# kiwicampus/multicamera_stitching

Hardware: NVIDIA B200
Metric: panoramas_per_sec (higher is better)
Workload: dtype u8

## Files before the change

multicamera_stitching_b200/csrc/mcs_stitch_tiled.cu:

```cuda
#include "mcs_device.cuh"

#include <cuda.h>
#include <string.h>
#include <stdlib.h>

#define TILED_WARPS MCS_TILED_WARPS
#define TILED_THREADS (32 * TILED_WARPS)
#define TILED_MIN_CTAS 2
#define TILED_PX_BATCH 4
#define TILED_SMEM_BUDGET_KB 113
#define TILED_MAX_STAGES 8
#define TILED_LOOKAHEAD_SLACK 2

struct TiledArgs {
    CUtensorMap tmap[MCS_MAX_LAYERS];
    const McsTile* tiles;
    const int4* issue;
    const McsLayer* layers;
    const uint32_t* desc;
    uint8_t* dst;
    long long dst_pitch;
    long long dst_frame_stride;
    int box_bytes;
    int stages;
    unsigned* work;
    int claim;
    int n_tiles;
    int n_chunks;
    int chunks_per_block;
    int split_first, split_end, split;
    int light_every, light_end, heavy_end, n_heavy;
    int frame_block;
    int nf_last;
    int n_blocks;
    int class_first[MCS_N_CLASSES + 1];
    int layer_sp[MCS_MAX_LAYERS];
    int layer_ox[MCS_MAX_LAYERS];
    const uint8_t* fast;
    int fast_stride;
    int fast_passes;
    int use_fast;
    const int4* band_issue;
    const uint32_t* band_desc;
    int feather_log2;
    int ov_bytes;
};

extern __shared__ __align__(128) uint8_t smem[];

__device__ __forceinline__ uint32_t smem_u32(const void* p) {
    return (uint32_t)__cvta_generic_to_shared(p);
}
__device__ __forceinline__ void mbar_init(uint32_t bar, int count) {
    asm volatile("mbarrier.init.shared::cta.b64 [%0], %1;" ::"r"(bar), "r"(count));
}
__device__ __forceinline__ void mbar_expect_tx(uint32_t bar, uint32_t bytes) {
    asm volatile("mbarrier.arrive.expect_tx.shared::cta.b64 _, [%0], %1;" ::"r"(bar), "r"(bytes) : "memory");
}
__device__ __forceinline__ void mbar_arrive(uint32_t bar) {
    asm volatile("mbarrier.arrive.shared::cta.b64 _, [%0];" ::"r"(bar) : "memory");
}
#ifdef TILED_DEBUG_HANG
#define TILED_HANG_CHECK(n_, what_)                                                                              \
    if (++(n_) > (1u << 26)) {                                                                                   \
        printf("tiled kernel stuck: %s line %d cta %d thread %d\n", what_, __LINE__, blockIdx.x, threadIdx.x);  \
        __trap();                                                                                                \
    }
#else
#define TILED_HANG_CHECK(n_, what_)
#endif
__device__ __forceinline__ void mbar_wait(uint32_t bar, uint32_t parity, int line = 0) {
    uint32_t done;
#ifdef TILED_DEBUG_HANG
    unsigned spins = 0;
#endif
    do {
        asm volatile(
            "{\n\t.reg .pred p;\n\t"
            "mbarrier.try_wait.parity.shared::cta.b64 p, [%1], %2;\n\t"
            "selp.u32 %0, 1, 0, p;\n\t}"
            : "=r"(done)
            : "r"(bar), "r"(parity)
            : "memory");
#ifdef TILED_DEBUG_HANG
        if (!done && ++spins > (1u << 22)) {
            printf("tiled kernel stuck: mbarrier wait from line %d cta %d thread %d bar %u parity %u\n", line, blockIdx.x,
                   threadIdx.x, bar, parity);
            __trap();
        }
#endif
    } while (!done);
}
__device__ __forceinline__ void tma_load_3d(uint32_t smem_dst, const CUtensorMap* map, int c0, int c1, int c2,
                                            uint32_t bar) {
    asm volatile(
        "cp.async.bulk.tensor.3d.shared::cluster.global.tile.mbarrier::complete_tx::bytes "
        "[%0], [%1, {%2, %3, %4}], [%5];" ::"r"(smem_dst),
        "l"(reinterpret_cast<uint64_t>(map)), "r"(c0), "r"(c1), "r"(c2), "r"(bar)
        : "memory");
}
__device__ __forceinline__ void bulk_g2s(uint32_t smem_dst, const void* src, uint32_t bytes, uint32_t bar) {
    asm volatile("cp.async.bulk.shared::cluster.global.mbarrier::complete_tx::bytes [%0], [%1], %2, [%3];" ::"r"(smem_dst),
                 "l"(src), "r"(bytes), "r"(bar)
                 : "memory");
}
__device__ __forceinline__ void cp_async16(uint32_t smem_dst, const void* src) {
    asm volatile("cp.async.ca.shared.global [%0], [%1], 16;" ::"r"(smem_dst), "l"(src) : "memory");
}
__device__ __forceinline__ void cp_async_wait_all() { asm volatile("cp.async.wait_all;" ::: "memory"); }
__device__ __forceinline__ uint32_t lds32(uint32_t addr) {
    uint32_t v;
    asm volatile("ld.shared.b32 %0, [%1];" : "=r"(v) : "r"(addr));
    return v;
}
__device__ __forceinline__ uint32_t lds32_box(uint32_t addr) {
    uint32_t v;
    asm("ld.shared.b32 %0, [%1];" : "=r"(v) : "r"(addr));
    return v;
}
__device__ __forceinline__ uint32_t order_after_wait(uint32_t addr) {
    asm volatile("" : "+r"(addr)::"memory");
    return addr;
}
__device__ __forceinline__ uint4 lds128(uint32_t addr) {
    uint4 v;
    asm volatile("ld.shared.v4.b32 {%0, %1, %2, %3}, [%4];" : "=r"(v.x), "=r"(v.y), "=r"(v.z), "=r"(v.w) : "r"(addr));
    return v;
}
__device__ __forceinline__ uint2 lds64(uint32_t addr) {
    uint2 v;
    asm volatile("ld.shared.v2.b32 {%0, %1}, [%2];" : "=r"(v.x), "=r"(v.y) : "r"(addr));
    return v;
}
__device__ __forceinline__ uint32_t lds8(uint32_t addr) {
    uint32_t v;
    asm volatile("ld.shared.u8 %0, [%1];" : "=r"(v) : "r"(addr));
    return v;
}
__device__ __forceinline__ uint32_t lds16(uint32_t addr) {
    uint32_t v;
    asm volatile("ld.shared.u16 %0, [%1];" : "=r"(v) : "r"(addr));
    return v;
}
__device__ __forceinline__ void sts8(uint32_t addr, uint32_t v) {
    asm volatile("st.shared.u8 [%0], %1;" ::"r"(addr), "r"(v) : "memory");
}
__device__ __forceinline__ void sts16(uint32_t addr, uint32_t v) {
    asm volatile("st.shared.u16 [%0], %1;" ::"r"(addr), "h"((unsigned short)v) : "memory");
}
__device__ __forceinline__ void sts32(uint32_t addr, uint32_t v) {
    asm volatile("st.shared.b32 [%0], %1;" ::"r"(addr), "r"(v) : "memory");
}
__device__ __forceinline__ uint32_t dp2a_lo(uint32_t w, uint32_t p, uint32_t acc) {
    uint32_t r;
    asm("dp2a.lo.u32.u32 %0, %1, %2, %3;" : "=r"(r) : "r"(w), "r"(p), "r"(acc));
    return r;
}
__device__ __forceinline__ uint32_t dp2a_hi(uint32_t w, uint32_t p, uint32_t acc) {
    uint32_t r;
    asm("dp2a.hi.u32.u32 %0, %1, %2, %3;" : "=r"(r) : "r"(w), "r"(p), "r"(acc));
    return r;
}
__device__ __forceinline__ uint32_t prmt(uint32_t a, uint32_t b, uint32_t sel) {
    uint32_t r;
    asm("prmt.b32 %0, %1, %2, %3;" : "=r"(r) : "r"(a), "r"(b), "r"(sel));
    return r;
}

#define MCS_STG128(p, v) __stcs((p), (v))

#define TILED_QD 32
#define TILED_SCHED_LEAD 10
struct SchedMem {
    int published;
    int pre_k;
    int pad[2];
    int4 pre;
    int4 pre_ov[MCS_BAND_MAX_OVERLAYS];
    int4 cur_ov[MCS_BAND_MAX_OVERLAYS];
// ... 239 lines not shown
        const uint32_t lo0 = __funnelshift_r(u0, u1, d.sh), lo1 = __funnelshift_r(v0, v1, d.sh);
        t[0] = dp2a_lo(d.w1, lo1, dp2a_lo(d.w0, lo0, 32768u));
    }
}

__device__ __forceinline__ PxDesc expand_desc(uint32_t w) {
    PxDesc d;
    const uint32_t b = w & 0xffffu, ax = (w >> 16) & 31u, ay = (w >> 21) & 31u;
    const uint32_t iax64 = (32u - ax) << 6, ax64 = ax << 6, iay = 32u - ay;
    d.off = b & ~3u;
    d.sh = b << 3;
    d.w0 = min(65535u, iay * iax64) | ((iay * ax64) << 16);
    d.w1 = (ay * iax64) | ((ay * ax64) << 16);
    return d;
}

struct RowOut {
    uint32_t s_chunk;
    uint32_t sh;
    uint32_t s_byte;
    uint32_t g_chunk;
    uint32_t g_byte;
    bool do_chunk, do_byte;
};

__device__ __forceinline__ RowOut row_split(uint32_t s_first, uint32_t g_first, uint32_t g_phase, bool has,
                                            int nbytes, int lane) {
    RowOut r;
    const int al = (int)((16u - g_phase) & 15u);
    const int head = min(nbytes, al);
    const int n = has ? (nbytes - head) >> 4 : 0;
    r.do_chunk = lane < n;
    r.s_chunk = s_first + al + (lane << 4);
    r.sh = 0;
    r.g_chunk = g_first + al + (lane << 4);
    const int e = lane < 16 ? lane : head + (n << 4) + lane - 16;
    r.do_byte = has && (lane < 16 ? lane < head : e < nbytes);
    r.s_byte = s_first + e;
    r.g_byte = g_first + e;
    return r;
}

__device__ __forceinline__ void write_out(const RowOut& r0, const RowOut& r1, bool ragged, uint8_t* frame) {
    const uint4 v0 = lds128(r0.s_chunk);
    const uint4 v1 = lds128(r1.s_chunk);
    if (r0.do_chunk) MCS_STG128(reinterpret_cast<uint4*>(frame + r0.g_chunk), v0);
    if (r1.do_chunk) MCS_STG128(reinterpret_cast<uint4*>(frame + r1.g_chunk), v1);
    if (ragged) {
        if (r0.do_byte) frame[r0.g_byte] = (uint8_t)lds8(r0.s_byte);
        if (r1.do_byte) frame[r1.g_byte] = (uint8_t)lds8(r1.s_byte);
    }
}

__device__ __forceinline__ void copy_out(const RowOut& r, uint32_t box, bool ragged, uint8_t* frame) {
    if (r.do_chunk) {
        const uint32_t w = box + r.s_chunk;
        const uint32_t w0 = lds32(w), w1 = lds32(w + 4), w2 = lds32(w + 8), w3 = lds32(w + 12), w4 = lds32(w + 16);
        uint4 v;
        v.x = __funnelshift_r(w0, w1, r.sh);
        v.y = __funnelshift_r(w1, w2, r.sh);
        v.z = __funnelshift_r(w2, w3, r.sh);
        v.w = __funnelshift_r(w3, w4, r.sh);
        MCS_STG128(reinterpret_cast<uint4*>(frame + r.g_chunk), v);
    }
    if (ragged && r.do_byte) frame[r.g_byte] = (uint8_t)lds8(box + r.s_byte);
}

template <int C>
__device__ __forceinline__ void stage_px(uint32_t o16, uint32_t o8, const uint32_t (&t)[C]) {
    if (C == 3) {
        sts16(o16, __byte_perm(t[0], t[1], 0x0062));
        sts8(o8, t[2] >> 16);
    } else {
#pragma unroll
        for (int k = 0; k < C; ++k) sts8(o16 + k, t[k] >> 16);
    }
}

#define TILED_SCHED_BYTES 640
static_assert(sizeof(SchedMem) <= TILED_SCHED_BYTES, "SchedMem must fit its shared-memory slot");

#define TILED_DESC_BUF_BYTES (MCS_FAST_HEADER_BYTES + MCS_CELL_W * MCS_CELL_H * 4)
static_assert(MCS_FAST_GROUP_BYTES + MCS_FAST_MAX_PASSES * MCS_FAST_PASS_BYTES <= MCS_CELL_W * MCS_CELL_H * 4,
              "a FAST record must fit the chunk-record buffer");

struct RingPos {
    int slot;
    uint32_t phase;
    int n;
    __device__ __forceinline__ void advance(int stages) {
        ++n;
        if (++slot == stages) { slot = 0; phase ^= 1; }
    }
};

struct Smem {
    uint32_t base;
    uint32_t out;
    uint32_t full;
    uint32_t empty;
    uint32_t dbar;
    uint32_t dbuf;
    uint32_t ov;
    SchedMem* issuer;
};

__device__ __forceinline__ void prefetch_chunk(const TiledArgs& a, const Smem& sm, int b, int4 e) {
    const int t = e.x;
    sts32(sm.dbar + 32 + 16 * b, (uint32_t)e.y);
    sts32(sm.dbar + 36 + 16 * b, (uint32_t)e.z);
    sts32(sm.dbar + 40 + 16 * b, (uint32_t)e.w);
    const int cls = tile_class(a, t);
    const uint32_t dst = sm.dbuf + b * TILED_DESC_BUF_BYTES, bar = sm.dbar + 8 * b;
    if (cls == MCS_TILE_FAST && a.use_fast) {
        mbar_expect_tx(bar, (uint32_t)a.fast_stride);
        bulk_g2s(dst, a.fast + (size_t)(t - a.class_first[1]) * a.fast_stride, (uint32_t)a.fast_stride, bar);
    } else if (cls >= MCS_TILE_WARP) {
        mbar_expect_tx(bar, 32u + MCS_CELL_W * MCS_CELL_H * 4u);
        bulk_g2s(dst, a.tiles + t, 32u, bar);
        bulk_g2s(dst + MCS_FAST_HEADER_BYTES, a.desc + (size_t)t * (MCS_CELL_W * MCS_CELL_H), MCS_CELL_W * MCS_CELL_H * 4u, bar);
    } else {
        mbar_expect_tx(bar, 32u);
        bulk_g2s(dst, a.tiles + t, 32u, bar);
    }
}

template <int C, int SP, bool ISS, bool BAND, bool BANDS>
__device__ __forceinline__ void warp_frames(const TiledArgs& a, const PxDesc (&d)[8], uint32_t groups, uint32_t sp,
                                            const Smem& sm, RingPos& ring, Issuer& issuer, int k_cons, uint8_t* frame,
                                            uint32_t g_row0, int n_fr, int c0, int nbytes, int h, int warp,
                                            int lane, int n_ov = 0, uint32_t ov_sp0 = 0, uint32_t ov_sp1 = 0,
                                            bool zero_base = false) {
    uint32_t ov_slots = 0;
    if (BAND) {
        for (int o = 0; o < n_ov; ++o)
#pragma unroll
            for (int j = 0; j < 8; ++j) {
                const uint32_t w = lds32(sm.ov + (uint32_t)o * (MCS_CELL_W * MCS_CELL_H * 4) + ((j * TILED_WARPS + warp) * 32 + lane) * 4);
                if (__any_sync(0xffffffffu, (w >> 26) != 0u)) ov_slots |= 1u << (8 * o + j);
            }
    }
    constexpr int OUT_PITCH = MCS_CELL_W * C + 16;
    const int stages = a.stages;
    const uint32_t g_row1 = g_row0 + (uint32_t)TILED_WARPS * (uint32_t)a.dst_pitch;
    const uint32_t s_row0 = sm.out + warp * OUT_PITCH, s_row1 = s_row0 + TILED_WARPS * OUT_PITCH;
    const bool has0 = warp < h, has1 = warp + TILED_WARPS < h;
    const bool phase_moves = (a.dst_frame_stride & 15) != 0;

    uint32_t ph0 = ((uint32_t)reinterpret_cast<uintptr_t>(frame) + g_row0) & 15u;
    uint32_t ph1 = ((uint32_t)reinterpret_cast<uintptr_t>(frame) + g_row1) & 15u;
    RowOut r0 = row_split(s_row0 + ph0 + c0 * C, g_row0 + c0 * C, (ph0 + c0 * C) & 15u, has0, nbytes, lane);
    RowOut r1 = row_split(s_row1 + ph1 + c0 * C, g_row1 + c0 * C, (ph1 + c0 * C) & 15u, has1, nbytes, lane);
    uint32_t st0 = s_row0 + ph0 + lane * C, st1 = s_row1 + ph1 + lane * C;
    uint32_t par = C == 3 ? (st0 & 1u) : 0u;
    TapSel sel = tap_sel<C>(par);
    bool ragged = __any_sync(0xffffffffu, r0.do_byte || r1.do_byte);

    for (int i = 0; i < n_fr; ++i, frame += a.dst_frame_stride) {
        if (ISS && lane == 0) issuer_step<BANDS, BAND>(a, sm.issuer, issuer, k_cons, ring.n, sm.base, sm.full, sm.empty);
        if (phase_moves && i != 0) {
            ph0 = ((uint32_t)reinterpret_cast<uintptr_t>(frame) + g_row0) & 15u;
            ph1 = ((uint32_t)reinterpret_cast<uintptr_t>(frame) + g_row1) & 15u;
            r0 = row_split(s_row0 + ph0 + c0 * C, g_row0 + c0 * C, (ph0 + c0 * C) & 15u, has0, nbytes, lane);
            r1 = row_split(s_row1 + ph1 + c0 * C, g_row1 + c0 * C, (ph1 + c0 * C) & 15u, has1, nbytes, lane);
            st0 = s_row0 + ph0 + lane * C;
            st1 = s_row1 + ph1 + lane * C;
            ragged = __any_sync(0xffffffffu, r0.do_byte || r1.do_byte);
            if (C == 3) {
                par = st0 & 1u;
                sel = tap_sel<C>(par);
            }
        }
        const uint32_t o16_0 = st0 + par, o8_0 = st0 + 2 - 2 * par;
        const uint32_t o16_1 = st1 + par, o8_1 = st1 + 2 - 2 * par;

        if (BAND && zero_base) {
            uint32_t z[C];
#pragma unroll
            for (int k = 0; k < C; ++k) z[k] = 0u;
#pragma unroll
            for (int j8 = 0; j8 < 8; ++j8) {
                const int g = 32 * (j8 & 3) * C;
                stage_px<C>((j8 < 4 ? o16_0 : o16_1) + g, (j8 < 4 ? o8_0 : o8_1) + g, z);
            }
            __syncwarp();
        } else {
        mbar_wait(sm.full + 8 * ring.slot, ring.phase, __LINE__);
        const uint32_t box = order_after_wait(sm.base + ring.slot * a.box_bytes);
        if (groups == 0xffu) {
#pragma unroll
            for (int b = 0; b < 8; b += TILED_PX_BATCH) {
                uint32_t t[TILED_PX_BATCH][C];
#pragma unroll
                for (int j = 0; j < TILED_PX_BATCH; ++j) sample_px<C, SP>(box, sp, d[b + j], sel, t[j]);
#pragma unroll
                for (int j = 0; j < TILED_PX_BATCH; ++j) {
                    const int g = 32 * ((b + j) & 3) * C;
                    stage_px<C>((b + j < 4 ? o16_0 : o16_1) + g, (b + j < 4 ? o8_0 : o8_1) + g, t[j]);
                }
            }
        } else {
#pragma unroll 1
            for (int jj = 0; jj < 4; ++jj) {
                if (!(groups & (0x11u << jj))) continue;
                uint32_t t0[C], t1[C];
                const PxDesc da = jj == 0 ? d[0] : jj == 1 ? d[1] : jj == 2 ? d[2] : d[3];
                const PxDesc db = jj == 0 ? d[4] : jj == 1 ? d[5] : jj == 2 ? d[6] : d[7];
                sample_px<C, SP>(box, sp, da, sel, t0);
                sample_px<C, SP>(box, sp, db, sel, t1);
                const int g = 32 * jj * C;
                stage_px<C>(o16_0 + g, o8_0 + g, t0);
                stage_px<C>(o16_1 + g, o8_1 + g, t1);
            }
        }
        __syncwarp();
        if (lane == 0) mbar_arrive(sm.empty + 8 * ring.slot);
        ring.advance(stages);
        }

        if (BAND) {
            const uint32_t F = 1u << a.feather_log2;
#pragma unroll 1
            for (int o = 0; o < n_ov; ++o) {
                if (ISS && lane == 0) issuer_step<BANDS, BAND>(a, sm.issuer, issuer, k_cons, ring.n, sm.base, sm.full, sm.empty);
                mbar_wait(sm.full + 8 * ring.slot, ring.phase, __LINE__);
                const uint32_t obox = order_after_wait(sm.base + ring.slot * a.box_bytes);
                const uint32_t osp = o == 0 ? ov_sp0 : ov_sp1;
                const uint32_t slab = sm.ov + (uint32_t)o * (MCS_CELL_W * MCS_CELL_H * 4) + (warp * 32 + lane) * 4;
#pragma unroll 1
                for (uint32_t todo = (ov_slots >> (8 * o)) & 0xffu; todo != 0u; todo &= todo - 1u) {
                    const int j = __ffs((int)todo) - 1;
                    const uint32_t w = lds32(slab + j * (TILED_WARPS * 32 * 4));
                    if (w >> 26) {
                        const uint32_t wa = (w >> 26) - 1u, wb = F - wa;
                        const PxDesc dd = expand_desc(w & 0x03ffffffu);
                        uint32_t t[C];
                        sample_px<C, 0>(obox, osp, dd, sel, t);
                        const int g = 32 * (j & 3) * C;
                        const uint32_t p16 = (j < 4 ? o16_0 : o16_1) + g, p8 = (j < 4 ? o8_0 : o8_1) + g;
                        uint32_t v[C];
                        if (C == 3) {
                            const uint32_t lo = lds16(p16);
                            v[0] = lo & 0xffu;
                            v[1 % C] = lo >> 8;
                            v[2 % C] = lds8(p8);
                        } else {
#pragma unroll
                            for (int k = 0; k < C; ++k) v[k] = lds8(p16 + k);
                        }
#pragma unroll
                        for (int k = 0; k < C; ++k)
                            t[k] = ((wa * v[k] + wb * ((t[k] >> 16) & 0xffu) + (F >> 1)) >> a.feather_log2) << 16;
                        stage_px<C>(p16, p8, t);
                    }
                }
                __syncwarp();
                if (lane == 0) mbar_arrive(sm.empty + 8 * ring.slot);
                ring.advance(stages);
            }
        }

        write_out(r0, r1, ragged, frame);
        __syncwarp();
    }
}

struct GroupDesc {
    uint32_t off;
    uint32_t sh;
    uint32_t w0[4];
    uint32_t w1[4];
};

__device__ __forceinline__ void tap_weights(uint32_t ax, uint32_t ay, uint32_t& w0, uint32_t& w1) {
    const uint32_t iax64 = (32u - ax) << 6, ax64 = ax << 6, iay = 32u - ay;
    w0 = min(65535u, iay * iax64) | ((iay * ax64) << 16);
    w1 = (ay * iax64) | ((ay * ax64) << 16);
}

__device__ __forceinline__ GroupDesc expand_group(uint2 g) {
    GroupDesc d;
    const uint32_t b = g.x & 0xffffu;
    d.off = b & ~3u;
    d.sh = (b & 3u) << 3;
    tap_weights((g.x >> 16) & 31u, (g.x >> 21) & 31u, d.w0[0], d.w1[0]);
#pragma unroll
    for (int j = 1; j < 4; ++j)
        tap_weights((g.y >> (10 * (j - 1))) & 31u, (g.y >> (10 * (j - 1) + 5)) & 31u, d.w0[j], d.w1[j]);
    return d;
}

__device__ __forceinline__ uint32_t pack4(uint32_t a, uint32_t b, uint32_t c, uint32_t d) {
    return prmt(prmt(a, b, 0x6262u), prmt(c, d, 0x6262u), 0x5410u);
}

template <int SP>
__device__ __forceinline__ void sample_group(uint32_t box, uint32_t sp, const GroupDesc& d, uint32_t (&out)[3]) {
    const uint32_t a0 = box + d.off;
    const uint32_t a1 = SP != 0 ? a0 + SP : a0 + sp;
    uint32_t u[5], v[5];
#pragma unroll
    for (int i = 0; i < 5; ++i) {
        u[i] = lds32_box(a0 + 4 * i);
        v[i] = lds32_box(a1 + 4 * i);
    }
    uint32_t A[4], B[4];
#pragma unroll
    for (int i = 0; i < 4; ++i) {
        A[i] = __funnelshift_r(u[i], u[i + 1], d.sh);
        B[i] = __funnelshift_r(v[i], v[i + 1], d.sh);
    }
    uint32_t t[4][3];
#define MCS_GROUP_PX(j, k, selp, kq, selq)                                                   \
    {                                                                                        \
        const uint32_t p0 = prmt(A[k], A[k + 1], selp), p1 = prmt(B[k], B[k + 1], selp);     \
        const uint32_t q0 = prmt(A[kq], A[kq + 1], selq), q1 = prmt(B[kq], B[kq + 1], selq); \
        t[j][0] = dp2a_lo(d.w1[j], p1, dp2a_lo(d.w0[j], p0, 32768u));                        \
        t[j][1] = dp2a_hi(d.w1[j], p1, dp2a_hi(d.w0[j], p0, 32768u));                        \
        t[j][2] = dp2a_lo(d.w1[j], q1, dp2a_lo(d.w0[j], q0, 32768u));                        \
    }
    MCS_GROUP_PX(0, 0, 0x4130u, 0, 0x5252u)
    MCS_GROUP_PX(1, 0, 0x7463u, 1, 0x4141u)
    MCS_GROUP_PX(2, 1, 0x6352u, 1, 0x7474u)
    MCS_GROUP_PX(3, 2, 0x5241u, 2, 0x6363u)
#undef MCS_GROUP_PX
    out[0] = pack4(t[0][0], t[0][1], t[0][2], t[1][0]);
    out[1] = pack4(t[1][1], t[1][2], t[2][0], t[2][1]);
    out[2] = pack4(t[2][2], t[3][0], t[3][1], t[3][2]);
}

struct GenDesc {
    PxDesc d;
    uint32_t pos;
};

__device__ __forceinline__ GenDesc expand_gen(uint2 e, int lane) {
    GenDesc g;
    g.d = expand_desc(e.x);
    const int rel = (int)(e.y & 127u) * 3 - lane * 12;
    g.pos = e.y == 0xffffffffu ? 0u : ((e.y & 128u) << 24) | 0x40000000u | ((uint32_t)rel & 0xffffu);
    return g;
}

template <int SP, bool ISS, bool BANDS>
__device__ __forceinline__ void fast_frames(const TiledArgs& a, const GroupDesc& g0, const GroupDesc& g1,
                                            const GenDesc (&gen)[MCS_FAST_MAX_PASSES], int n_pass, uint32_t sp,
                                            const Smem& sm, RingPos& ring, Issuer& issuer, int k_cons, uint8_t* frame,
                                            uint32_t g_row0, int n_fr, int c0, int nbytes, int h, int warp,
                                            int lane) {
    constexpr int C = 3;
    constexpr int OUT_PITCH = MCS_CELL_W * C + 16;
    const int stages = a.stages;
    const TapSel sel = tap_sel<C>(0u);
    RowOut r0, r1;
    uint32_t st0, st1;
    bool ragged;
    {
        const uint32_t g_row1 = g_row0 + (uint32_t)TILED_WARPS * (uint32_t)a.dst_pitch;
        const uint32_t s_row0 = sm.out + warp * OUT_PITCH, s_row1 = s_row0 + TILED_WARPS * OUT_PITCH;
        const uint32_t ph0 = ((uint32_t)reinterpret_cast<uintptr_t>(frame) + g_row0) & 15u;
        const uint32_t ph1 = ((uint32_t)reinterpret_cast<uintptr_t>(frame) + g_row1) & 15u;
        r0 = row_split(s_row0 + ph0 + c0 * C, g_row0 + c0 * C, (ph0 + c0 * C) & 15u, warp < h, nbytes, lane);
        r1 = row_split(s_row1 + ph1 + c0 * C, g_row1 + c0 * C, (ph1 + c0 * C) & 15u, warp + TILED_WARPS < h, nbytes,
                       lane);
        st0 = s_row0 + ph0 + lane * (4 * C);
        st1 = s_row1 + ph1 + lane * (4 * C);
        ragged = __any_sync(0xffffffffu, r0.do_byte || r1.do_byte);
    }
    for (int i = 0; i < n_fr; ++i, frame += a.dst_frame_stride) {
        if (ISS && lane == 0) issuer_step<BANDS, false>(a, sm.issuer, issuer, k_cons, ring.n, sm.base, sm.full, sm.empty);
        mbar_wait(sm.full + 8 * ring.slot, ring.phase, __LINE__);
        const uint32_t box = order_after_wait(sm.base + ring.slot * a.box_bytes);
        {
            uint32_t o0[3], o1[3];
            sample_group<SP>(box, sp, g0, o0);
            sample_group<SP>(box, sp, g1, o1);
            sts32(st0, o0[0]); sts32(st0 + 4, o0[1]); sts32(st0 + 8, o0[2]);
            sts32(st1, o1[0]); sts32(st1 + 4, o1[1]); sts32(st1 + 8, o1[2]);
        }
        if (n_pass > 0) {
            __syncwarp();
#pragma unroll
            for (int p = 0; p < MCS_FAST_MAX_PASSES; ++p) {
                if (p < n_pass) {
                    uint32_t t[C];
                    sample_px<C, SP>(box, sp, gen[p].d, sel, t);
                    const uint32_t o = ((int)gen[p].pos < 0 ? st1 : st0) + (uint32_t)(int)(short)gen[p].pos;
                    if (gen[p].pos & 0x40000000u) {
                        sts8(o, t[0] >> 16);
                        sts8(o + 1, t[1] >> 16);
                        sts8(o + 2, t[2] >> 16);
                    }
                }
            }
        }
        __syncwarp();
        if (lane == 0) mbar_arrive(sm.empty + 8 * ring.slot);
        ring.advance(stages);

        write_out(r0, r1, ragged, frame);
        __syncwarp();
    }
}

template <int C, bool BANDS>
__global__ void __launch_bounds__(TILED_THREADS, TILED_MIN_CTAS)
mcs_stitch_tiled_kernel(const __grid_constant__ TiledArgs a) {
    constexpr int OUT_PITCH = MCS_CELL_W * C + 16;
    const int stages = a.stages;
    Smem sm;
    sm.base = smem_u32(smem);
    sm.full = sm.base + stages * a.box_bytes;
    sm.empty = sm.full + 8 * TILED_MAX_STAGES;
    sm.issuer = reinterpret_cast<SchedMem*>(smem + stages * a.box_bytes + 16 * TILED_MAX_STAGES);
    sm.dbar = sm.empty + 8 * TILED_MAX_STAGES + TILED_SCHED_BYTES;
    sm.out = sm.dbar + 64;
    sm.dbuf = (sm.out + MCS_CELL_H * OUT_PITCH + 15u) & ~15u;
    sm.ov = sm.dbuf + 2 * TILED_DESC_BUF_BYTES + 1024;
    asm volatile("" : "+r"(sm.base), "+r"(sm.full), "+r"(sm.empty), "+r"(sm.out));

    const int tid = threadIdx.x, warp = tid >> 5, lane = tid & 31;
    Issuer issuer;
    issuer_init(sm.issuer, issuer, tid == 0);
    if (tid == 0) {
        for (int s = 0; s < stages; ++s) {
            mbar_init(sm.full + 8 * s, 1);
            mbar_init(sm.empty + 8 * s, TILED_WARPS);
        }
        for (int b = 0; b < 2; ++b) {
            mbar_init(sm.dbar + 8 * b, 1);
            mbar_init(sm.dbar + 16 + 8 * b, TILED_WARPS);
        }
        if (BANDS) {
            mbar_init(sm.ov + a.ov_bytes, 1);
            mbar_init(sm.ov + a.ov_bytes + 8, TILED_WARPS);
        }
        asm volatile("fence.mbarrier_init.release.cluster;" ::: "memory");
        asm volatile("fence.proxy.async.shared::cta;" ::: "memory");
    }
    __syncthreads();

    if (tid == 0) {
        sched_ensure(a, sm.issuer, issuer, 2);
        const int4 e0 = sm.issuer->chunk[0];
        if (e0.x >= 0) prefetch_chunk(a, sm, 0, e0);
        for (int i = 0; i < stages - TILED_LOOKAHEAD_SLACK; ++i)
            issuer_step<BANDS, BANDS>(a, sm.issuer, issuer, BANDS ? -1 : 0, -1, sm.base, sm.full, sm.empty);
    }

    RingPos ring{0, 0u, 0};
    if (BANDS && lane == 0) sts32(sm.ov + a.ov_bytes + 16 + 4 * warp, 0u);
    const uint32_t s_published = smem_u32(&sm.issuer->published), s_ids = smem_u32(&sm.issuer->chunk[0]);
    for (int k_cons = 0;; ++k_cons) {
        const int cb = k_cons & 1;
        const uint32_t rec = sm.dbuf + cb * TILED_DESC_BUF_BYTES;
        const uint32_t rec_release = sm.dbar + 16 + 8 * cb;
        if (tid == 0) {
            sched_ensure(a, sm.issuer, issuer, k_cons + 2);
            int4 e2 = make_int4(-1, 0, 0, 0);
            if (k_cons + 1 < issuer.claimed) e2 = sm.issuer->chunk[(k_cons + 1) % TILED_QD];
            if (e2.x >= 0) {
                if (k_cons >= 1) mbar_wait(sm.dbar + 16 + 8 * (cb ^ 1), (uint32_t)(((k_cons - 1) >> 1) & 1), __LINE__);
                prefetch_chunk(a, sm, cb ^ 1, e2);
            }
        }
        {
#ifdef TILED_DEBUG_HANG
            unsigned spins = 0;
#endif
            while (ld_volatile_shared(s_published) <= k_cons) { TILED_HANG_CHECK(spins, "waiting for a chunk id") }
        }
        const int id = ld_volatile_shared(s_ids + 16 * (k_cons % TILED_QD));
        if (id < 0) break;
        mbar_wait(sm.dbar + 8 * cb, (uint32_t)((k_cons >> 1) & 1), __LINE__);
        const uint4 info = lds128(sm.dbar + 32 + 16 * cb);
        const int blk = (int)info.x, f0 = (int)info.y, f1 = (int)info.z;
        McsTile tile;
        {
            const uint4 q0 = lds128(rec), q1 = lds128(rec + 16);
            tile.cx0 = (int)q0.x;
            tile.y0 = (int)q0.y;
            tile.c0 = (short)(q0.z & 0xffffu);
            tile.c1 = (short)(q0.z >> 16);
            tile.h = (short)(q0.w & 0xffffu);
            tile.layer = (short)(q0.w >> 16);
            tile.cls = (short)(q1.x & 0xffffu);
            tile.flags = (short)(q1.x >> 16);
            tile.bx = (int)q1.y;
            tile.by = (int)q1.z;
            tile.reserved = (int)q1.w;
        }
        const int c0 = tile.c0, c1 = tile.c1, h = tile.h;
        const int nbytes = (c1 - c0) * C;
        const int n_fr = f1 - f0;
        uint8_t* const frame0 = a.dst + ((long long)blk * a.frame_block + f0) * a.dst_frame_stride;
        const uint32_t g_cell = (uint32_t)tile.y0 * (uint32_t)a.dst_pitch + (uint32_t)(tile.cx0 * C);
        const bool phase_moves = (a.dst_frame_stride & 15) != 0;

        if (tile.cls == MCS_TILE_ZERO || tile.cls == MCS_TILE_COPY) {
            __syncwarp();
            if (lane == 0) mbar_arrive(rec_release);
        }
        if (tile.cls == MCS_TILE_ZERO) {
            const uint32_t g_first0 = g_cell + (uint32_t)warp * (uint32_t)a.dst_pitch + c0 * C;
            const uint32_t g_first1 = g_first0 + (uint32_t)TILED_WARPS * (uint32_t)a.dst_pitch;
            uint8_t* frame = frame0;
            RowOut r0, r1;
            for (int i = 0; i < n_fr; ++i, frame += a.dst_frame_stride) {
                if (warp == 0 && lane == 0) issuer_step<BANDS, false>(a, sm.issuer, issuer, k_cons, ring.n, sm.base, sm.full, sm.empty);
                if (i == 0 || phase_moves) {
                    const uint32_t fp = (uint32_t)reinterpret_cast<uintptr_t>(frame);
                    r0 = row_split(0, g_first0, (fp + g_first0) & 15u, warp < h, nbytes, lane);
                    r1 = row_split(0, g_first1, (fp + g_first1) & 15u, warp + TILED_WARPS < h, nbytes, lane);
                }
                const uint4 z = make_uint4(0u, 0u, 0u, 0u);
                if (r0.do_chunk) MCS_STG128(reinterpret_cast<uint4*>(frame + r0.g_chunk), z);
                if (r1.do_chunk) MCS_STG128(reinterpret_cast<uint4*>(frame + r1.g_chunk), z);
                if (r0.do_byte) frame[r0.g_byte] = 0;
                if (r1.do_byte) frame[r1.g_byte] = 0;
            }
            continue;
        }
        const uint32_t sp = (uint32_t)a.layer_sp[tile.layer];

        if (tile.cls == MCS_TILE_COPY) {
            const uint32_t s_off = (uint32_t)((tile.cx0 + c0 - a.layer_ox[tile.layer]) * C - 4 * tile.bx);
            const uint32_t g_first0 = g_cell + (uint32_t)warp * (uint32_t)a.dst_pitch + c0 * C;
            const uint32_t g_first1 = g_first0 + (uint32_t)TILED_WARPS * (uint32_t)a.dst_pitch;
            uint8_t* frame = frame0;
            RowOut r0, r1;
            bool ragged = false;
            for (int i = 0; i < n_fr; ++i, frame += a.dst_frame_stride) {
                if (warp == 0 && lane == 0) issuer_step<BANDS, false>(a, sm.issuer, issuer, k_cons, ring.n, sm.base, sm.full, sm.empty);
                if (i == 0 || phase_moves) {
                    const uint32_t fp = (uint32_t)reinterpret_cast<uintptr_t>(frame);
                    r0 = row_split(s_off + warp * sp, g_first0, (fp + g_first0) & 15u, warp < h, nbytes, lane);
                    r1 = row_split(s_off + (warp + TILED_WARPS) * sp, g_first1, (fp + g_first1) & 15u,
                                   warp + TILED_WARPS < h, nbytes, lane);
                    r0.sh = (r0.s_chunk & 3u) * 8u; r0.s_chunk &= ~3u;
                    r1.sh = (r1.s_chunk & 3u) * 8u; r1.s_chunk &= ~3u;
                    ragged = __any_sync(0xffffffffu, r0.do_byte || r1.do_byte);
                }
                mbar_wait(sm.full + 8 * ring.slot, ring.phase, __LINE__);
                const uint32_t box = sm.base + ring.slot * a.box_bytes;
                copy_out(r0, box, ragged, frame);
                copy_out(r1, box, ragged, frame);
                __syncwarp();
                if (lane == 0) mbar_arrive(sm.empty + 8 * ring.slot);
                ring.advance(stages);
            }
            continue;
        }

        const uint32_t g_row0 = g_cell + (uint32_t)warp * (uint32_t)a.dst_pitch;
        int n_ov = 0;
        uint32_t ov_sp0 = 0, ov_sp1 = 0;
        bool zero_base = false;
        if (BANDS && tile.cls == MCS_TILE_BAND) {
            n_ov = (tile.reserved >> 24) & 15;
            zero_base = ((tile.reserved >> 28) & 1) != 0;
            const uint32_t ov_full = sm.ov + a.ov_bytes, ov_empty = ov_full + 8;
            const int band_seq = (int)lds32(ov_full + 16 + 4 * warp);
            if (tid == 0) {
                if (band_seq > 0) mbar_wait(ov_empty, (uint32_t)((band_seq - 1) & 1), __LINE__);
                mbar_expect_tx(ov_full, (uint32_t)n_ov * (MCS_CELL_W * MCS_CELL_H * 4u));
                bulk_g2s(sm.ov, a.band_desc + (size_t)id * (MCS_BAND_MAX_OVERLAYS * MCS_CELL_W * MCS_CELL_H),
                         (uint32_t)n_ov * (MCS_CELL_W * MCS_CELL_H * 4u), ov_full);
            }
            const int4 r0 = __ldg(a.band_issue + id * (1 + MCS_BAND_MAX_OVERLAYS) + 1);
            const int4 r1 = __ldg(a.band_issue + id * (1 + MCS_BAND_MAX_OVERLAYS) + 2);
            ov_sp0 = (uint32_t)a.layer_sp[r0.x];
            ov_sp1 = r1.x >= 0 ? (uint32_t)a.layer_sp[r1.x] : 0u;
            if (tid == 0)
                for (int i = 0; i < stages - TILED_LOOKAHEAD_SLACK; ++i)
                    issuer_step<BANDS, BANDS>(a, sm.issuer, issuer, k_cons, ring.n, sm.base, sm.full, sm.empty);
            mbar_wait(ov_full, (uint32_t)(band_seq & 1), __LINE__);
            __syncwarp();
            if (lane == 0) sts32(ov_full + 16 + 4 * warp, (uint32_t)(band_seq + 1));
        }
        if (C == 3 && tile.cls == MCS_TILE_FAST && a.use_fast) {
            const uint32_t grp = rec + MCS_FAST_HEADER_BYTES;
            const uint32_t lst = rec + MCS_FAST_HEADER_BYTES + MCS_FAST_GROUP_BYTES;
            const uint2 w0 = lds64(grp + (warp * 32 + lane) * 8), w1 = lds64(grp + ((TILED_WARPS + warp) * 32 + lane) * 8);
            const int n_pass = ((int)lds8(rec + 32 + warp) + 31) >> 5;
            GenDesc gen[MCS_FAST_MAX_PASSES];
#pragma unroll
            for (int p = 0; p < MCS_FAST_MAX_PASSES; ++p) {
                uint2 e = make_uint2(0u, 0xffffffffu);
                if (p < n_pass) e = lds64(lst + ((p * TILED_WARPS + warp) * 32 + lane) * 8);
                gen[p] = expand_gen(e, lane);
            }
            __syncwarp();
            if (lane == 0) mbar_arrive(rec_release);
            const GroupDesc g0 = expand_group(w0), g1 = expand_group(w1);
            const int n_call = phase_moves ? n_fr : 1, fr_call = phase_moves ? 1 : n_fr;
#define MCS_FAST_FRAMES(SP_, ISS_)                                                                                  \
    for (int q = 0; q < n_call; ++q)                                                                                  \
        fast_frames<SP_, ISS_, BANDS>(a, g0, g1, gen, n_pass, sp, sm, ring, issuer, k_cons,                                 \
                               frame0 + (long long)q * a.dst_frame_stride, g_row0, fr_call, c0, nbytes, h, warp, lane)
            if (warp == 0) {
                if (sp == 512) MCS_FAST_FRAMES(512, true); else MCS_FAST_FRAMES(0, true);
            } else {
                if (sp == 512) MCS_FAST_FRAMES(512, false); else MCS_FAST_FRAMES(0, false);
            }
#undef MCS_FAST_FRAMES
            continue;
        }

        PxDesc d[8];
        {
            const uint32_t dp = rec + MCS_FAST_HEADER_BYTES + (warp * 32 + lane) * 4;
            uint32_t w[8];
#pragma unroll
            for (int j = 0; j < 8; ++j) w[j] = lds32(dp + j * (TILED_WARPS * 32 * 4));
            __syncwarp();
            if (lane == 0) mbar_arrive(rec_release);
#pragma unroll
            for (int j = 0; j < 8; ++j) d[j] = expand_desc(w[j]);
        }
        uint32_t groups = 0;
#pragma unroll
        for (int j = 0; j < 8; ++j) {
            const int row = warp + TILED_WARPS * (j >> 2), g0c = 32 * (j & 3);
            if (row < h && g0c < c1 && g0c + 32 > c0) groups |= 1u << j;
        }
        constexpr int SP_MAIN = C == 1 ? 256 : C == 3 ? 512 : 640;
#define MCS_WARP_FRAMES(SP_, ISS_, BAND_)                                                                           \
    warp_frames<C, SP_, ISS_, BAND_, BANDS>(a, d, groups, sp, sm, ring, issuer, k_cons, frame0, g_row0, n_fr, c0, nbytes, h, \
                                     warp, lane, n_ov, ov_sp0, ov_sp1, zero_base)
        if (BANDS && tile.cls == MCS_TILE_BAND) {
            if (warp == 0) MCS_WARP_FRAMES(0, true, BANDS); else MCS_WARP_FRAMES(0, false, BANDS);
            __syncwarp();
            if (lane == 0) mbar_arrive(sm.ov + a.ov_bytes + 8);
        } else if (warp == 0) {
            if (sp == SP_MAIN) MCS_WARP_FRAMES(SP_MAIN, true, false); else MCS_WARP_FRAMES(0, true, false);
        } else {
            if (sp == SP_MAIN) MCS_WARP_FRAMES(SP_MAIN, false, false); else MCS_WARP_FRAMES(0, false, false);
        }
#undef MCS_WARP_FRAMES
    }
    if (tid == 0) {
        __threadfence();
        if (atomicAdd(a.work + 1, 1u) == gridDim.x - 1) {
            a.work[0] = 0u;
            a.work[1] = 0u;
            __threadfence();
        }
    }
}

typedef CUresult (*EncodeTiledFn)(CUtensorMap*, CUtensorMapDataType, cuuint32_t, void*, const cuuint64_t*,
                                  const cuuint64_t*, const cuuint32_t*, const cuuint32_t*, CUtensorMapInterleave,
                                  CUtensorMapSwizzle, CUtensorMapL2promotion, CUtensorMapFloatOOBfill);

static EncodeTiledFn get_encode_fn() {
    static EncodeTiledFn fn = nullptr;
    static bool tried = false;
    if (!tried) {
        tried = true;
        void* p = nullptr;
        cudaDriverEntryPointQueryResult q;
        if (cudaGetDriverEntryPoint("cuTensorMapEncodeTiled", &p, cudaEnableDefault, &q) == cudaSuccess &&
            q == cudaDriverEntryPointSuccess)
            fn = reinterpret_cast<EncodeTiledFn>(p);
    }
    return fn;
}

static size_t tiled_ov_bytes(const mcs_plan* plan) {
    return plan->band_fused && plan->n_band > 0 ? (size_t)plan->band_max_ov * MCS_CELL_W * MCS_CELL_H * 4 : 0;
}

static size_t tiled_smem_bytes(const mcs_plan* plan, int stages) {
    const int out_pitch = MCS_CELL_W * plan->channels + 16;
    return (size_t)stages * plan->box_bytes + 2 * TILED_MAX_STAGES * sizeof(uint64_t) + TILED_SCHED_BYTES +
           64  + (size_t)MCS_CELL_H * out_pitch + 16 + 2 * TILED_DESC_BUF_BYTES + 1024 +
           (tiled_ov_bytes(plan) ? tiled_ov_bytes(plan) + 64 : 0);
}

static int tiled_stages(const mcs_plan* plan) {
    const size_t budget = (size_t)TILED_SMEM_BUDGET_KB * 1024;
    int s = TILED_MAX_STAGES;
    while (s > 3 && tiled_smem_bytes(plan, s) > budget) --s;
    return s;
}

const char* mcs_tiled_blocker(const mcs_plan* plan, const uint8_t* const* src, const int64_t* pitch,
                              const int64_t* fstride, int n_frames, int64_t dst_pitch) {
    if (!plan->tiled_ok) return plan->tiled_why;
    if (dst_pitch <= 0 || (long long)plan->out_h * dst_pitch >= (1ll << 32))
        return "output frame of 4 GiB or more (the tiled kernel addresses a frame with 32-bit offsets)";
    if (!get_encode_fn()) return "cuTensorMapEncodeTiled unavailable";
    if (plan->rows_need_pad && !plan->pad_promised)
        return "a source row is not a multiple of 4 bytes (zero-padded rows were not promised)";
    for (int k = 0; k < plan->n_layers; ++k) {
        if (pitch[k] < (((int64_t)plan->layers[k].src_w * plan->channels + 3) & ~(int64_t)3))
            return "source pitch smaller than the row rounded up to 4 bytes";
        if ((reinterpret_cast<uintptr_t>(src[k]) & 15) != 0) return "source base not 16-byte aligned";
        if ((pitch[k] & 15) != 0) return "source pitch not a multiple of 16 bytes";
        if (n_frames > 1 && (fstride[k] & 15) != 0) return "source frame stride not a multiple of 16 bytes";
        if (n_frames > 1 && fstride[k] <= 0) return "non-positive source frame stride";
    }
    return nullptr;
}

int mcs_launch_tiled(mcs_plan* plan, const uint8_t* const* src, const int64_t* pitch, const int64_t* fstride,
                     int n_frames, uint8_t* dst, int64_t dst_pitch, int64_t dst_frame_stride,
                     cudaStream_t stream) {
    TiledArgs a;
    memset(&a, 0, sizeof(a));
    bool hit = plan->cache_valid && plan->cache_frames == n_frames;
    for (int k = 0; hit && k < plan->n_layers; ++k)
        hit = plan->cache_src[k] == src[k] && plan->cache_pitch[k] == pitch[k] &&
              (n_frames == 1 || plan->cache_fstride[k] == fstride[k]);
    CUtensorMap* cache = reinterpret_cast<CUtensorMap*>(
        (reinterpret_cast<uintptr_t>(plan->tmap_cache) + 63) & ~(uintptr_t)63);
    if (!hit) {
        EncodeTiledFn enc = get_encode_fn();
        for (int k = 0; k < plan->n_layers; ++k) {
            const McsLayer& L = plan->layers[k];
            const cuuint64_t dims[3] = {(cuuint64_t)((L.src_w * plan->channels + 3) / 4), (cuuint64_t)L.src_h,
                                        (cuuint64_t)n_frames};
            const cuuint64_t strides[2] = {(cuuint64_t)pitch[k],
                                           (cuuint64_t)(n_frames > 1 ? fstride[k] : pitch[k] * L.src_h)};
            const cuuint32_t box[3] = {(cuuint32_t)L.bw4, (cuuint32_t)L.bh, 1u};
            const cuuint32_t estr[3] = {1u, 1u, 1u};
            CUresult r = enc(&cache[k], CU_TENSOR_MAP_DATA_TYPE_UINT32, 3, const_cast<uint8_t*>(src[k]), dims,
                             strides, box, estr, CU_TENSOR_MAP_INTERLEAVE_NONE, CU_TENSOR_MAP_SWIZZLE_NONE,
                             CU_TENSOR_MAP_L2_PROMOTION_L2_128B, CU_TENSOR_MAP_FLOAT_OOB_FILL_NONE);
// ... 49 lines not shown
            return MCS_ERR_UNSUPPORTED;
        }
        plan->grid_ctas_per_sm = per_sm;
        plan->n_sm = n_sm;
    }
    const int fb = plan->frame_block < n_frames ? plan->frame_block : n_frames;
    a.frame_block = fb;
    a.n_blocks = (n_frames + fb - 1) / fb;
    a.nf_last = n_frames - (a.n_blocks - 1) * fb;

    long long grid = (long long)plan->n_sm * plan->grid_ctas_per_sm;
    const long long units = (long long)plan->n_tiles * fb;
    if (grid > units) grid = units;
    a.n_tiles = plan->n_tiles;
    a.split_end = plan->class_first[MCS_SEG(MCS_TILE_COPY)];
    a.split = fb >= 16 ? 4 : 1;
    const int split_tiles = 2 * (int)grid;
    {
        const char* env = getenv("MCS_TILED_SPLIT");
        if (env) a.split = atoi(env) > 1 && fb >= atoi(env) ? atoi(env) : 1;
    }
    if (a.split > 1 && a.nf_last < a.split) a.split = 1;
    a.split_first = a.split > 1 ? (a.split_end > split_tiles ? a.split_end - split_tiles : 0) : a.split_end;
    a.chunks_per_block = plan->n_tiles + (a.split_end - a.split_first) * (a.split - 1);
    {
        const int n_light = plan->n_tiles - a.split_end, n_heavy = a.chunks_per_block - n_light;
        a.n_heavy = n_heavy;
        a.light_every = n_light > 0 ? n_heavy / n_light + 1 : 2;
        if (a.light_every < 2) a.light_every = 2;
        int zone = n_light < n_heavy / (a.light_every - 1) ? n_light : n_heavy / (a.light_every - 1);
        a.light_end = zone * a.light_every;
        a.heavy_end = n_heavy + a.light_end / a.light_every;
    }
    if ((long long)a.n_blocks * a.chunks_per_block >= (1ll << 30)) {
        mcs_set_error("mcs_stitch_u8: %d frame blocks x %d chunks exceed the chunk counter", a.n_blocks, a.chunks_per_block);
        return MCS_ERR_UNSUPPORTED;
    }
    a.n_chunks = a.n_blocks * a.chunks_per_block;
    {
        int claim = 32 / fb;
        const long long fair = a.n_chunks / (4 * grid);
        if (claim > fair) claim = (int)fair;
        a.claim = claim < 1 ? 1 : claim > 8 ? 8 : claim;
    }
    a.work = plan->d_work;
    for (int c = 0; c <= MCS_N_CLASSES; ++c) a.class_first[c] = plan->class_first[c];
    a.band_issue = plan->d_band_issue;
    a.band_desc = plan->d_band_desc;
    a.feather_log2 = plan->feather_log2;
    a.ov_bytes = (int)tiled_ov_bytes(plan);
    a.fast = plan->d_fast;
    a.fast_stride = plan->fast_stride;
    a.fast_passes = plan->fast_passes;
    a.use_fast = plan->d_fast != nullptr && (reinterpret_cast<uintptr_t>(dst) & 3) == 0 && (dst_pitch & 3) == 0 &&
                 (n_frames == 1 || (dst_frame_stride & 3) == 0);
    kern<<<(unsigned)grid, TILED_THREADS, smem, stream>>>(a);
    mcs_count_launch(1);
    MCS_CHECK_CUDA(cudaGetLastError());
    return MCS_OK;
}
```

Measured before the change: 60270.

## Stage BGR pixels as 4-byte words and write output with aligned 32-bit stores

For 3-channel tiles outside feathered bands with 4-aligned columns and 4-byte-aligned output rows, pixels are staged in shared memory as padded 32-bit words. Each lane then packs four pixels into three 32-bit streaming stores, replacing the byte-phase row_split, ragged-byte and 16-byte-store path. The shared-memory staging layout, the smem size accounting (the 1024-byte slack is dropped) and the copy/zero tile paths are also reworked, with row splits now recomputed every frame. The trade is 4-byte stores instead of 16-byte ones, plus extra template instantiations and code size.

New measurement: 60740 (median of 6 runs). About the same (+0.8%).

```diff
diff --git a/multicamera_stitching_b200/csrc/mcs_stitch_tiled.cu b/multicamera_stitching_b200/csrc/mcs_stitch_tiled.cu
--- a/multicamera_stitching_b200/csrc/mcs_stitch_tiled.cu
+++ b/multicamera_stitching_b200/csrc/mcs_stitch_tiled.cu
@@ -39,6 +39,7 @@
     const uint8_t* fast;
     int fast_stride;
     int fast_passes;
+    int rows4;
     int use_fast;
     const int4* band_issue;
     const uint32_t* band_desc;
@@ -125,6 +126,16 @@
 __device__ __forceinline__ uint4 lds128(uint32_t addr) {
     uint4 v;
     asm volatile("ld.shared.v4.b32 {%0, %1, %2, %3}, [%4];" : "=r"(v.x), "=r"(v.y), "=r"(v.z), "=r"(v.w) : "r"(addr));
+    return v;
+}
+__device__ __forceinline__ uint4 lds128_if(uint32_t addr, bool on) {
+    uint4 v;
+    asm volatile(
+        "{\n\t.reg .pred p;\n\t"
+        "setp.ne.b32 p, %5, 0;\n\t"
+        "@p ld.shared.v4.b32 {%0, %1, %2, %3}, [%4];\n\t}"
+        : "=r"(v.x), "=r"(v.y), "=r"(v.z), "=r"(v.w)
+        : "r"(addr), "r"((uint32_t)on));
     return v;
 }
 __device__ __forceinline__ uint2 lds64(uint32_t addr) {
@@ -470,6 +481,16 @@
     }
 }
 
+__device__ __forceinline__ void write_out_words(uint32_t s, uint8_t* g, bool on) {
+    const uint4 v = lds128_if(s, on);
+    if (on) {
+        unsigned* p = reinterpret_cast<unsigned*>(g);
+        __stcs(p, prmt(v.x, v.y, 0x4210u));
+        __stcs(p + 1, prmt(v.y, v.z, 0x5421u));
+        __stcs(p + 2, prmt(v.z, v.w, 0x6542u));
+    }
+}
+
 __device__ __forceinline__ void copy_out(const RowOut& r, uint32_t box, bool ragged, uint8_t* frame) {
     if (r.do_chunk) {
         const uint32_t w = box + r.s_chunk;
@@ -494,6 +515,14 @@
         for (int k = 0; k < C; ++k) sts8(o16 + k, t[k] >> 16);
     }
 }
+
+template <int C>
+__device__ __forceinline__ void stage_word(uint32_t o, const uint32_t (&t)[C]) {
+    sts32(o, prmt(prmt(t[0], t[1 % C], 0x0062u), t[2 % C], 0x0610u));
+}
+
+#define TILED_OUT_PITCH(C) ((C) == 3 ? MCS_CELL_W * 4 : MCS_CELL_W * (C) + 16)
+#define TILED_STAGING_BYTES(C) ((C) == 3 ? MCS_CELL_H * MCS_CELL_W * 4 : MCS_CELL_H * TILED_OUT_PITCH(C) + 16)
 
 #define TILED_SCHED_BYTES 640
 static_assert(sizeof(SchedMem) <= TILED_SCHED_BYTES, "SchedMem must fit its shared-memory slot");
@@ -543,7 +572,7 @@
     }
 }
 
-template <int C, int SP, bool ISS, bool BAND, bool BANDS>
+template <int C, int SP, bool ISS, bool BAND, bool BANDS, bool WORDS>
 __device__ __forceinline__ void warp_frames(const TiledArgs& a, const PxDesc (&d)[8], uint32_t groups, uint32_t sp,
                                             const Smem& sm, RingPos& ring, Issuer& issuer, int k_cons, uint8_t* frame,
                                             uint32_t g_row0, int n_fr, int c0, int nbytes, int h, int warp,
@@ -558,25 +587,32 @@
                 if (__any_sync(0xffffffffu, (w >> 26) != 0u)) ov_slots |= 1u << (8 * o + j);
             }
     }
-    constexpr int OUT_PITCH = MCS_CELL_W * C + 16;
+    static_assert(!WORDS || (C == 3 && !BAND), "word staging is for BGR pixels outside BAND tiles");
+    constexpr int OUT_PITCH = TILED_OUT_PITCH(C);
+    constexpr int PX_BYTES = WORDS ? 4 : C;
     const int stages = a.stages;
     const uint32_t g_row1 = g_row0 + (uint32_t)TILED_WARPS * (uint32_t)a.dst_pitch;
     const uint32_t s_row0 = sm.out + warp * OUT_PITCH, s_row1 = s_row0 + TILED_WARPS * OUT_PITCH;
     const bool has0 = warp < h, has1 = warp + TILED_WARPS < h;
-    const bool phase_moves = (a.dst_frame_stride & 15) != 0;
-
-    uint32_t ph0 = ((uint32_t)reinterpret_cast<uintptr_t>(frame) + g_row0) & 15u;
-    uint32_t ph1 = ((uint32_t)reinterpret_cast<uintptr_t>(frame) + g_row1) & 15u;
+    const bool phase_moves = !WORDS && (a.dst_frame_stride & 15) != 0;
+
+    uint32_t ph0 = WORDS ? 0u : ((uint32_t)reinterpret_cast<uintptr_t>(frame) + g_row0) & 15u;
+    uint32_t ph1 = WORDS ? 0u : ((uint32_t)reinterpret_cast<uintptr_t>(frame) + g_row1) & 15u;
     RowOut r0 = row_split(s_row0 + ph0 + c0 * C, g_row0 + c0 * C, (ph0 + c0 * C) & 15u, has0, nbytes, lane);
     RowOut r1 = row_split(s_row1 + ph1 + c0 * C, g_row1 + c0 * C, (ph1 + c0 * C) & 15u, has1, nbytes, lane);
-    uint32_t st0 = s_row0 + ph0 + lane * C, st1 = s_row1 + ph1 + lane * C;
-    uint32_t par = C == 3 ? (st0 & 1u) : 0u;
+    uint32_t st0 = s_row0 + ph0 + lane * PX_BYTES, st1 = s_row1 + ph1 + lane * PX_BYTES;
+    uint32_t par = C == 3 && !WORDS ? (st0 & 1u) : 0u;
     TapSel sel = tap_sel<C>(par);
-    bool ragged = __any_sync(0xffffffffu, r0.do_byte || r1.do_byte);
+    bool ragged = !WORDS && __any_sync(0xffffffffu, r0.do_byte || r1.do_byte);
+    uint32_t wl = (uint32_t)lane;
+    asm volatile("" : "+r"(wl));
+    const bool won = (int)(4 * wl) >= c0 && (int)(4 * wl) < c0 + nbytes / C;
+    const bool won0 = has0 && won, won1 = has1 && won;
+    const uint32_t wg0 = g_row0 + 12 * wl, wo0 = st0 + 12 * wl;
 
     for (int i = 0; i < n_fr; ++i, frame += a.dst_frame_stride) {
         if (ISS && lane == 0) issuer_step<BANDS, BAND>(a, sm.issuer, issuer, k_cons, ring.n, sm.base, sm.full, sm.empty);
-        if (phase_moves && i != 0) {
+        if (!WORDS && phase_moves && i != 0) {
             ph0 = ((uint32_t)reinterpret_cast<uintptr_t>(frame) + g_row0) & 15u;
             ph1 = ((uint32_t)reinterpret_cast<uintptr_t>(frame) + g_row1) & 15u;
             r0 = row_split(s_row0 + ph0 + c0 * C, g_row0 + c0 * C, (ph0 + c0 * C) & 15u, has0, nbytes, lane);
@@ -613,8 +649,9 @@
                 for (int j = 0; j < TILED_PX_BATCH; ++j) sample_px<C, SP>(box, sp, d[b + j], sel, t[j]);
 #pragma unroll
                 for (int j = 0; j < TILED_PX_BATCH; ++j) {
-                    const int g = 32 * ((b + j) & 3) * C;
-                    stage_px<C>((b + j < 4 ? o16_0 : o16_1) + g, (b + j < 4 ? o8_0 : o8_1) + g, t[j]);
+                    const int g = 32 * ((b + j) & 3) * PX_BYTES;
+                    if constexpr (WORDS) stage_word<C>((b + j < 4 ? st0 : st1) + g, t[j]);
+                    else stage_px<C>((b + j < 4 ? o16_0 : o16_1) + g, (b + j < 4 ? o8_0 : o8_1) + g, t[j]);
                 }
             }
         } else {
@@ -626,9 +663,14 @@
                 const PxDesc db = jj == 0 ? d[4] : jj == 1 ? d[5] : jj == 2 ? d[6] : d[7];
                 sample_px<C, SP>(box, sp, da, sel, t0);
                 sample_px<C, SP>(box, sp, db, sel, t1);
-                const int g = 32 * jj * C;
-                stage_px<C>(o16_0 + g, o8_0 + g, t0);
-                stage_px<C>(o16_1 + g, o8_1 + g, t1);
+                const int g = 32 * jj * PX_BYTES;
+                if constexpr (WORDS) {
+                    stage_word<C>(st0 + g, t0);
+                    stage_word<C>(st1 + g, t1);
+                } else {
+                    stage_px<C>(o16_0 + g, o8_0 + g, t0);
+                    stage_px<C>(o16_1 + g, o8_1 + g, t1);
+                }
             }
         }
         __syncwarp();
@@ -678,7 +720,12 @@
             }
         }
 
-        write_out(r0, r1, ragged, frame);
+        if constexpr (WORDS) {
+            write_out_words(wo0, frame + wg0, won0);
+            write_out_words(wo0 + TILED_WARPS * OUT_PITCH, frame + wg0 + (uint32_t)TILED_WARPS * (uint32_t)a.dst_pitch, won1);
+        }
+        else
+            write_out(r0, r1, ragged, frame);
         __syncwarp();
     }
 }
@@ -767,7 +814,7 @@
                                             uint32_t g_row0, int n_fr, int c0, int nbytes, int h, int warp,
                                             int lane) {
     constexpr int C = 3;
-    constexpr int OUT_PITCH = MCS_CELL_W * C + 16;
+    constexpr int OUT_PITCH = TILED_OUT_PITCH(C);
     const int stages = a.stages;
     const TapSel sel = tap_sel<C>(0u);
     RowOut r0, r1;
@@ -824,7 +871,6 @@
 template <int C, bool BANDS>
 __global__ void __launch_bounds__(TILED_THREADS, TILED_MIN_CTAS)
 mcs_stitch_tiled_kernel(const __grid_constant__ TiledArgs a) {
-    constexpr int OUT_PITCH = MCS_CELL_W * C + 16;
     const int stages = a.stages;
     Smem sm;
     sm.base = smem_u32(smem);
@@ -833,9 +879,9 @@
     sm.issuer = reinterpret_cast<SchedMem*>(smem + stages * a.box_bytes + 16 * TILED_MAX_STAGES);
     sm.dbar = sm.empty + 8 * TILED_MAX_STAGES + TILED_SCHED_BYTES;
     sm.out = sm.dbar + 64;
-    sm.dbuf = (sm.out + MCS_CELL_H * OUT_PITCH + 15u) & ~15u;
-    sm.ov = sm.dbuf + 2 * TILED_DESC_BUF_BYTES + 1024;
-    asm volatile("" : "+r"(sm.base), "+r"(sm.full), "+r"(sm.empty), "+r"(sm.out));
+    sm.dbuf = sm.out + TILED_STAGING_BYTES(C);
+    sm.ov = sm.dbuf + 2 * TILED_DESC_BUF_BYTES;
+    asm volatile("" : "+r"(sm.base), "+r"(sm.full), "+r"(sm.empty));
 
     const int tid = threadIdx.x, warp = tid >> 5, lane = tid & 31;
     Issuer issuer;
@@ -923,14 +969,11 @@
             const uint32_t g_first0 = g_cell + (uint32_t)warp * (uint32_t)a.dst_pitch + c0 * C;
             const uint32_t g_first1 = g_first0 + (uint32_t)TILED_WARPS * (uint32_t)a.dst_pitch;
             uint8_t* frame = frame0;
-            RowOut r0, r1;
             for (int i = 0; i < n_fr; ++i, frame += a.dst_frame_stride) {
                 if (warp == 0 && lane == 0) issuer_step<BANDS, false>(a, sm.issuer, issuer, k_cons, ring.n, sm.base, sm.full, sm.empty);
-                if (i == 0 || phase_moves) {
-                    const uint32_t fp = (uint32_t)reinterpret_cast<uintptr_t>(frame);
-                    r0 = row_split(0, g_first0, (fp + g_first0) & 15u, warp < h, nbytes, lane);
-                    r1 = row_split(0, g_first1, (fp + g_first1) & 15u, warp + TILED_WARPS < h, nbytes, lane);
-                }
+                const uint32_t fp = (uint32_t)reinterpret_cast<uintptr_t>(frame);
+                const RowOut r0 = row_split(0, g_first0, (fp + g_first0) & 15u, warp < h, nbytes, lane);
+                const RowOut r1 = row_split(0, g_first1, (fp + g_first1) & 15u, warp + TILED_WARPS < h, nbytes, lane);
                 const uint4 z = make_uint4(0u, 0u, 0u, 0u);
                 if (r0.do_chunk) MCS_STG128(reinterpret_cast<uint4*>(frame + r0.g_chunk), z);
                 if (r1.do_chunk) MCS_STG128(reinterpret_cast<uint4*>(frame + r1.g_chunk), z);
@@ -944,25 +987,21 @@
         if (tile.cls == MCS_TILE_COPY) {
             const uint32_t s_off = (uint32_t)((tile.cx0 + c0 - a.layer_ox[tile.layer]) * C - 4 * tile.bx);
             const uint32_t g_first0 = g_cell + (uint32_t)warp * (uint32_t)a.dst_pitch + c0 * C;
-            const uint32_t g_first1 = g_first0 + (uint32_t)TILED_WARPS * (uint32_t)a.dst_pitch;
             uint8_t* frame = frame0;
-            RowOut r0, r1;
-            bool ragged = false;
             for (int i = 0; i < n_fr; ++i, frame += a.dst_frame_stride) {
                 if (warp == 0 && lane == 0) issuer_step<BANDS, false>(a, sm.issuer, issuer, k_cons, ring.n, sm.base, sm.full, sm.empty);
-                if (i == 0 || phase_moves) {
-                    const uint32_t fp = (uint32_t)reinterpret_cast<uintptr_t>(frame);
-                    r0 = row_split(s_off + warp * sp, g_first0, (fp + g_first0) & 15u, warp < h, nbytes, lane);
-                    r1 = row_split(s_off + (warp + TILED_WARPS) * sp, g_first1, (fp + g_first1) & 15u,
-                                   warp + TILED_WARPS < h, nbytes, lane);
-                    r0.sh = (r0.s_chunk & 3u) * 8u; r0.s_chunk &= ~3u;
-                    r1.sh = (r1.s_chunk & 3u) * 8u; r1.s_chunk &= ~3u;
-                    ragged = __any_sync(0xffffffffu, r0.do_byte || r1.do_byte);
-                }
                 mbar_wait(sm.full + 8 * ring.slot, ring.phase, __LINE__);
                 const uint32_t box = sm.base + ring.slot * a.box_bytes;
-                copy_out(r0, box, ragged, frame);
-                copy_out(r1, box, ragged, frame);
+#pragma unroll
+                for (int rr = 0; rr < 2; ++rr) {
+                    const int row = warp + rr * TILED_WARPS;
+                    const uint32_t g_first = g_first0 + (uint32_t)(rr * TILED_WARPS) * (uint32_t)a.dst_pitch;
+                    RowOut r = row_split(s_off + row * sp, g_first, ((uint32_t)reinterpret_cast<uintptr_t>(frame) + g_first) & 15u,
+                                         row < h, nbytes, lane);
+                    r.sh = (r.s_chunk & 3u) * 8u;
+                    r.s_chunk &= ~3u;
+                    copy_out(r, box, __any_sync(0xffffffffu, r.do_byte), frame);
+                }
                 __syncwarp();
                 if (lane == 0) mbar_arrive(sm.empty + 8 * ring.slot);
                 ring.advance(stages);
@@ -1043,17 +1082,26 @@
             if (row < h && g0c < c1 && g0c + 32 > c0) groups |= 1u << j;
         }
         constexpr int SP_MAIN = C == 1 ? 256 : C == 3 ? 512 : 640;
-#define MCS_WARP_FRAMES(SP_, ISS_, BAND_)                                                                           \
-    warp_frames<C, SP_, ISS_, BAND_, BANDS>(a, d, groups, sp, sm, ring, issuer, k_cons, frame0, g_row0, n_fr, c0, nbytes, h, \
-                                     warp, lane, n_ov, ov_sp0, ov_sp1, zero_base)
+#define MCS_WARP_FRAMES(SP_, ISS_, BAND_, WORDS_)                                                                   \
+    warp_frames<C, SP_, ISS_, BAND_, BANDS, WORDS_>(a, d, groups, sp, sm, ring, issuer, k_cons, frame0, g_row0, n_fr, c0, \
+                                                    nbytes, h, warp, lane, n_ov, ov_sp0, ov_sp1, zero_base)
+        const bool words = C == 3 && !BANDS && sp == SP_MAIN && a.rows4 && ((c0 | c1) & 3) == 0;
         if (BANDS && tile.cls == MCS_TILE_BAND) {
-            if (warp == 0) MCS_WARP_FRAMES(0, true, BANDS); else MCS_WARP_FRAMES(0, false, BANDS);
+            if (warp == 0) MCS_WARP_FRAMES(0, true, BANDS, false); else MCS_WARP_FRAMES(0, false, BANDS, false);
             __syncwarp();
             if (lane == 0) mbar_arrive(sm.ov + a.ov_bytes + 8);
+        } else if (C == 3) {
+            if constexpr (C == 3) {
+                if (words) {
+                    if (warp == 0) MCS_WARP_FRAMES(SP_MAIN, true, false, true); else MCS_WARP_FRAMES(SP_MAIN, false, false, true);
+                } else {
+                    if (warp == 0) MCS_WARP_FRAMES(0, true, false, false); else MCS_WARP_FRAMES(0, false, false, false);
+                }
+            }
         } else if (warp == 0) {
-            if (sp == SP_MAIN) MCS_WARP_FRAMES(SP_MAIN, true, false); else MCS_WARP_FRAMES(0, true, false);
+            if (sp == SP_MAIN) MCS_WARP_FRAMES(SP_MAIN, true, false, false); else MCS_WARP_FRAMES(0, true, false, false);
         } else {
-            if (sp == SP_MAIN) MCS_WARP_FRAMES(SP_MAIN, false, false); else MCS_WARP_FRAMES(0, false, false);
+            if (sp == SP_MAIN) MCS_WARP_FRAMES(SP_MAIN, false, false, false); else MCS_WARP_FRAMES(0, false, false, false);
         }
 #undef MCS_WARP_FRAMES
     }
@@ -1090,9 +1138,8 @@
 }
 
 static size_t tiled_smem_bytes(const mcs_plan* plan, int stages) {
-    const int out_pitch = MCS_CELL_W * plan->channels + 16;
     return (size_t)stages * plan->box_bytes + 2 * TILED_MAX_STAGES * sizeof(uint64_t) + TILED_SCHED_BYTES +
-           64  + (size_t)MCS_CELL_H * out_pitch + 16 + 2 * TILED_DESC_BUF_BYTES + 1024 +
+           64  + TILED_STAGING_BYTES(plan->channels) + 2 * TILED_DESC_BUF_BYTES +
            (tiled_ov_bytes(plan) ? tiled_ov_bytes(plan) + 64 : 0);
 }
 
@@ -1248,8 +1295,9 @@
     a.fast = plan->d_fast;
     a.fast_stride = plan->fast_stride;
     a.fast_passes = plan->fast_passes;
-    a.use_fast = plan->d_fast != nullptr && (reinterpret_cast<uintptr_t>(dst) & 3) == 0 && (dst_pitch & 3) == 0 &&
-                 (n_frames == 1 || (dst_frame_stride & 3) == 0);
+    a.rows4 = (reinterpret_cast<uintptr_t>(dst) & 3) == 0 && (dst_pitch & 3) == 0 &&
+              (n_frames == 1 || (dst_frame_stride & 3) == 0);
+    a.use_fast = plan->d_fast != nullptr && a.rows4;
     kern<<<(unsigned)grid, TILED_THREADS, smem, stream>>>(a);
     mcs_count_launch(1);
     MCS_CHECK_CUDA(cudaGetLastError());
```
